# microsoft/UniVL

Measured on AMD Instinct MI355X. Metric: video-text pairs/sec (retrieval finetune, 48x48), higher is better.
Workload: dtype bf16; 1 GPU; YouCookII-shape retrieval finetune (FT-Joint) training step: BERT-base text encoder (12 L) + 6-layer visual encoder, max_words=48, max_frames=48, bs=4 per GPU, fwd+bwd+clip+BertAdam, dropout 0.10, random-init weights; kind=joint, per_gpu_batch=4, global_batch=4, max_words=48, max_frames=48, parallelism=dp1, hip_graph=True, graph_mode=whole, optimizer_pipelined=True, optimizer_riding=True, params=152602880

## Files before the change

### univl_amd/csrc/gemm.hip

```cpp
#include <stdlib.h>
#include "common.h"
#include "univl_hip.h"
#include "adam_body.h"
#include "ln_body.h"

#ifdef UNIVL_TRACE
__device__ unsigned long long* g_univl_trace = nullptr;
__device__ int g_univl_trace_cap = 0;
#define UNIVL_TRACE_AT(phase)                                                                              \
    do {                                                                                                   \
        if (threadIdx.x == 0 && g_univl_trace != nullptr) {                                                \
            const int w__ = blockIdx.x + gridDim.x * (blockIdx.y + gridDim.y * blockIdx.z);                \
            if (w__ < g_univl_trace_cap) g_univl_trace[w__ * 4 + (phase)] = wall_clock64();                \
        }                                                                                                  \
    } while (0)
extern "C" int univl_trace_set(unsigned long long* buf, int cap_workgroups) {
    if (hipMemcpyToSymbol(HIP_SYMBOL(g_univl_trace), &buf, sizeof(buf)) != hipSuccess) return 1;
    if (hipMemcpyToSymbol(HIP_SYMBOL(g_univl_trace_cap), &cap_workgroups, sizeof(int)) != hipSuccess) return 1;
    return 0;
}
#else
#define UNIVL_TRACE_AT(phase)
#endif

// ... 711 lines not shown
    fold_leave(cnt);
}

__host__ __device__ __forceinline__ void pair_tile(int t, int total, int nx, int ny, int nz, int flags, int gm, int& bx, int& by, int& bz) {
    if ((flags & UNIVL_GEMM_XCD_MAP) && total >= 16 && ny > 1) {
        tile_of(xcd_run(t, total), nx, ny, nz, gm, bx, by, bz);
    } else {
        const int nxy = nx * ny;
        bz = t / nxy;
        const int rem = t - bz * nxy;
        by = rem / nx;
        bx = rem - by * nx;
    }
}

template <bool DR, int WF, bool FOLD = false>
__global__ __launch_bounds__(512, (DR && WF == 2 && !FOLD) ? 6 : 4) void gemm_pair_kernel(PairArgs a, LnFold f) {
    const int w0 = blockIdx.x;
    int bx, by, bz;
    if (w0 < a.nd_pad) {
        if (w0 >= a.nd) return;
        pair_tile(w0, a.nd, a.dnx, a.dny, a.dnz, a.d.flags, a.d.gm, bx, by, bz);
        if constexpr (DR) gemm_tile<__bf16, false, true, 64, 128, 2, 2, 4>(a.d, bx, by, bz, a.dnz);
        else gemm_tile<__bf16, false, true, 64, 64, 4, 2, 4>(a.d, bx, by, bz, a.dnz);
        if constexpr (FOLD) ln_fold_bwd(f, by, a.dnx * a.dnz);
    } else if (w0 < a.nd_pad + a.cs.n_pad) {
        const int t = w0 - a.nd_pad;
        if (t >= a.cs.n_tiles) return;
        colsum_tile<512>(a.cs, t, smem_raw);
    } else {
        pair_tile(w0 - a.nd_pad - a.cs.n_pad, a.nw, a.wnx, a.wny, a.wnz, a.w.flags, a.w.gm, bx, by, bz);
        if constexpr (WF == 0) gemm_tile<__bf16, true, true, 64, 64, 4, 2, 4>(a.w, bx, by, bz, a.wnz);
        else if constexpr (WF == 1) gemm_tile<__bf16, true, true, 64, 64, 6, 2, 4>(a.w, bx, by, bz, a.wnz);
        else if constexpr (WF == 2) gemm_tile<__bf16, true, true, 128, 64, 2, 4, 2>(a.w, bx, by, bz, a.wnz);
        else gemm_tile<__bf16, true, true, 128, 64, 6, 4, 2>(a.w, bx, by, bz, a.wnz);
    }
}

template <bool DR, int WF, bool FOLD = false>
int launch_pair(const PairArgs& a, hipStream_t stream, const LnFold* f = nullptr) {
    constexpr size_t smem_d = DR ? 2 * (size_t)(64 + 128) * 64 * sizeof(__bf16) : 2 * (size_t)(64 + 64) * 128 * sizeof(__bf16);
    constexpr size_t smem_w = WF == 0 ? 2 * (size_t)(64 + 64) * 128 * sizeof(__bf16)
                              : WF == 1 ? (size_t)(64 + 64) * 192 * sizeof(__bf16)
                              : WF == 2 ? 2 * (size_t)(128 + 64) * 64 * sizeof(__bf16) : (size_t)(128 + 64) * 192 * sizeof(__bf16);
    constexpr size_t smem = smem_d > smem_w ? smem_d : smem_w;
    static_assert(!FOLD || smem >= 8 * 768 * sizeof(float), "LayerNorm-backward fold needs 24 KB of LDS");
    static bool attr_done[UNIVL_MAX_DEVICES] = {};
    univl_allow_lds(gemm_pair_kernel<DR, WF, FOLD>, smem, attr_done);
    LnFold none = {};
    hipLaunchKernelGGL((gemm_pair_kernel<DR, WF, FOLD>), dim3(a.nd_pad + a.cs.n_pad + a.nw), dim3(512), smem, stream, a, f ? *f : none);
    UNIVL_LAUNCH_CHECK();
    return UNIVL_OK;
}

template <typename T, bool TA, bool TB, int BM, int BN, int NC, int WGM, int WGN>
__device__ __forceinline__ void gemm_acc_only(const T* A, long lda, const T* B, long ldb, int M, int N, int K, int m0, int n0,
                                              f32x4_t (&acc)[BM / WGM / 16][BN / WGN / 16], unsigned char* smem) {
    constexpr int BK = NC * Mma<T>::CH, NT = 64 * WGM * WGN;
    using TileA = Tile<T, TA, BM, BK, NT>;
    using TileB = Tile<T, TB, BN, BK, NT>;
    constexpr int WM = BM / WGM, WN = BN / WGN, MI = WM / 16, NI = WN / 16;
    unsigned char* sA = smem;
    unsigned char* sB = sA + 2 * TileA::BYTES;
    const int tid = threadIdx.x, lane = tid & 63, wave = tid >> 6;
    const int wm0 = (wave / WGN) * WM, wn0 = (wave % WGN) * WN;
#pragma unroll
    for (int a = 0; a < MI; ++a)
#pragma unroll
        for (int b = 0; b < NI; ++b) acc[a][b] = f32x4_t{0.f, 0.f, 0.f, 0.f};
    const T* pa[TileA::PER_THREAD];
    const T* pb[TileB::PER_THREAD];
    TileA::init(pa, A, lda, m0, 0, M, tid);
    TileB::init(pb, B, ldb, n0, 0, N, tid);
    const long stepA = TileA::kstep(lda), stepB = TileB::kstep(ldb);
    const int nfull = K / BK;
    TileA::issue(pa, sA, tid);
    TileB::issue(pb, sB, tid);
    TileA::advance(pa, stepA);
    TileB::advance(pb, stepB);
    __syncthreads();
    for (int t = 0; t < nfull; ++t) {
        const int cur = t & 1;
        if (t + 1 < nfull) {
            TileA::issue(pa, sA + (cur ^ 1) * TileA::BYTES, tid);
            TileB::issue(pb, sB + (cur ^ 1) * TileB::BYTES, tid);
            TileA::advance(pa, stepA);
            TileB::advance(pb, stepB);
        }
        tile_mma<T, TA, TB, MI, NI, NC, TileA, TileB>(sA + cur * TileA::BYTES, sB + cur * TileB::BYTES, wm0, wn0, lane, acc);
        __syncthreads();
    }
}

#include "vocab_ce.h"
#include "vocab_score.h"
#include "attn_body.h"

struct AttnFusedArgs {
    UnivlAttention at;
    int Sk_pad, Sq_pad;
    const __bf16* dY; long lddy;
    const __bf16* W; long ldw;
    int K;
    int n_attn, n_attn_pad;
    GemmArgs w;
    int nw, wnx, wny, wnz;
};

template <int TRIPS, bool DUAL, int NCW>
__global__ __launch_bounds__(256) void attn_bwd_odgrad_kernel(AttnFusedArgs a) {
    const int w0 = blockIdx.x;
    if (w0 < a.n_attn_pad) {
        if (w0 >= a.n_attn) return;
        const int bh = w0 >> 1, role = w0 & 1;
        const int b = bh / a.at.H, h = bh % a.at.H;
        f32x4_t acc[2][2];
        gemm_acc_only<__bf16, false, true, 64, 64, 4, 2, 2>(a.dY + (long)b * a.at.Sq * a.lddy, a.lddy, a.W, a.ldw, a.at.Sq, a.at.H * 64, a.K,
                                                            0, h * 64, acc, smem_raw);
        const int lane = threadIdx.x & 63, wave = threadIdx.x >> 6, g = lane >> 4, i = lane & 15;
        const int wm0 = (wave >> 1) * 32, wn0 = (wave & 1) * 32;
        const int Sq = a.at.Sq, Sq_pad = a.Sq_pad;
        auto dow = [&](void* img_, int pitch) {
            __bf16* img = reinterpret_cast<__bf16*>(img_);
#pragma unroll
            for (int ta = 0; ta < 2; ++ta)
#pragma unroll
                for (int tb = 0; tb < 2; ++tb)
#pragma unroll
                    for (int r = 0; r < 4; ++r) {
                        const int row = wm0 + 16 * ta + 4 * g + r, col = wn0 + 16 * tb + i;
                        if (row < Sq_pad) img[row * pitch + col] = row < Sq ? (__bf16)acc[ta][tb][r] : (__bf16)0.0f;
                    }
        };
        attn_bwd_body<__bf16, TRIPS, DUAL, true>(a.at, a.Sk_pad, a.Sq_pad, 1, 0.125f, bh, role, smem_raw, dow);
    } else {
        int bx, by, bz;
        pair_tile(w0 - a.n_attn_pad, a.nw, a.wnx, a.wny, a.wnz, a.w.flags, a.w.gm, bx, by, bz);
        gemm_tile<__bf16, true, true, 64, 64, NCW, 2, 2>(a.w, bx, by, bz, a.wnz);
    }
}

struct AttnFwdFusedArgs {
    UnivlAttention at;
    int Sk_pad;
    const __bf16* X; long ldx;
    const __bf16* W; long ldw;
    const float* bias;
    __bf16* qkv; long ldqkv;
    int K;
    int n_attn, n_attn_pad;
    const __bf16* X_lo; const __bf16* W_lo;
};

template <bool NT, bool BIG>
__global__ __launch_bounds__(512, 2) void attn_fwd_qkv_kernel(AttnFwdFusedArgs a, UnivlAdam ad, int c0, int c1) {
    const int w0 = blockIdx.x;
    if (w0 >= a.n_attn_pad) {
        const int nb = (int)gridDim.x - a.n_attn_pad;
        for (int c = c0 + (w0 - a.n_attn_pad); c < c1; c += nb) adam_chunk<NT, 512>(ad, c);
        return;
    }
    if (w0 >= a.n_attn) return;
    constexpr int ROWS = BIG ? 128 : 64, MI = ROWS / 32;
    using TileA = Tile<__bf16, false, ROWS, 64, 512>;
    using TileB = Tile<__bf16, false, 192, 64, 512>;
    const int bh = BIG ? (w0 >> 1) : w0, yblk = BIG ? (w0 & 1) : 0, b = bh / a.at.H, h = bh % a.at.H;
    const int HD3 = a.at.H * 64, Sq = a.at.Sq;
    const int tid = threadIdx.x, lane = tid & 63, wave = tid >> 6, g = lane >> 4, i = lane & 15;
    const int wm0 = (wave >> 2) * (ROWS / 2), wn0 = (wave & 3) * 48;
    unsigned char* sA = smem_raw;
    unsigned char* sB = sA + 2 * TileA::BYTES;
    f32x4_t acc[MI][3];
#pragma unroll
    for (int ta = 0; ta < MI; ++ta)
#pragma unroll
        for (int tb = 0; tb < 3; ++tb) acc[ta][tb] = f32x4_t{0.f, 0.f, 0.f, 0.f};
    const __bf16* pa[TileA::PER_THREAD];
    const __bf16* pb[TileB::PER_THREAD];
    TileA::init(pa, a.X + (long)b * Sq * a.ldx, a.ldx, 0, 0, Sq, tid);
#pragma unroll
    for (int c = 0; c < TileB::PER_THREAD; ++c) {
        int r, q;
        TileB::coords(c, tid, r, q);
        pb[c] = a.W + (long)((r >> 6) * HD3 + h * 64 + (r & 63)) * a.ldw + q * 8;
    }
    const int nseg = 1 + (a.W_lo != nullptr ? 1 : 0) + (a.X_lo != nullptr ? 1 : 0);
    const int per = a.K / 64, nfull = nseg * per;
    int seg = 0, wrap = per;
    auto seg_x = [&](int s_) { return (a.X_lo != nullptr && s_ > 0 && s_ == nseg - 1) ? a.X_lo : a.X; };
    auto seg_w = [&](int s_) { return (a.W_lo != nullptr && s_ == 1) ? a.W_lo : a.W; };
    TileA::issue(pa, sA, tid);
    TileB::issue(pb, sB, tid);
    TileA::advance(pa, 64);
    TileB::advance(pb, 64);
    __syncthreads();
    for (int t = 0; t < nfull; ++t) {
        const int cur = t & 1;
        if (t + 1 < nfull) {
            if (t + 1 == wrap) {
                TileA::advance(pa, (seg_x(seg + 1) - seg_x(seg)) - (long)a.K);
                TileB::advance(pb, (seg_w(seg + 1) - seg_w(seg)) - (long)a.K);
                ++seg;
                wrap += per;
            }
            TileA::issue(pa, sA + (cur ^ 1) * TileA::BYTES, tid);
            TileB::issue(pb, sB + (cur ^ 1) * TileB::BYTES, tid);
            TileA::advance(pa, 64);
            TileB::advance(pb, 64);
        }
        tile_mma<__bf16, false, false, MI, 3, 2, TileA, TileB>(sA + cur * TileA::BYTES, sB + cur * TileB::BYTES, wm0, wn0, lane, acc);
        __syncthreads();
    }
    const AttnFwdImages<__bf16> im(smem_raw, a.Sk_pad);
    using C = AttnCfg<__bf16>;
#pragma unroll
    for (int tb = 0; tb < 3; ++tb) {
        const int col = wn0 + 16 * tb + i, panel = col >> 6, c64 = col & 63;
        const int gcol = panel * HD3 + h * 64 + c64;
        const float bv = a.bias ? a.bias[gcol] : 0.0f;
        __bf16* img = panel == 0 ? im.sQ : (panel == 1 ? im.sK : im.sV);
        const int pitch = panel == 2 ? C::PT : C::PK;
#pragma unroll
        for (int ta = 0; ta < MI; ++ta)
#pragma unroll
            for (int r = 0; r < 4; ++r) {
                const int row = wm0 + 16 * ta + 4 * g + r;
                const __bf16 v = (__bf16)(acc[ta][tb][r] * 1.0f + bv);
                if (row < Sq && (!BIG || (row >> 6) == yblk)) a.qkv[((long)b * Sq + row) * a.ldqkv + gcol] = v;
                if (row < a.Sk_pad || (!BIG && panel == 0)) img[row * pitch + c64] = row < Sq ? v : (__bf16)0.0f;
            }
    }
    attn_fwd_body<__bf16, BIG ? 8 : 4, true>(a.at, a.Sk_pad, 0.125f, bh, yblk, smem_raw);
}

template <bool NT>
__global__ __launch_bounds__(512, 2) void gemm_adam_kernel(GemmArgs g, int nd, int nd_pad, int nx, int ny, int nz, UnivlAdam a, int c0, int c1) {
    const int w0 = blockIdx.x;
    if (w0 < nd_pad) {
        if (w0 >= nd) return;
        int bx, by, bz;
        pair_tile(w0, nd, nx, ny, nz, g.flags, g.gm, bx, by, bz);
        gemm_tile<__bf16, false, false, 64, 64, 4, 2, 4, true>(g, bx, by, bz, nz);
    } else {
        const int nb = (int)gridDim.x - nd_pad;
        for (int c = c0 + (w0 - nd_pad); c < c1; c += nb) adam_chunk<NT, 512>(a, c);
    }
}

__host__ __device__ __forceinline__ bool rect_rider_role(int w0, int total, int nd_pad, int& idx) {
    const int gi = w0 >> 3, nrg = (total - nd_pad) >> 3, pg = (total >> 3) / nrg;
    const int k = gi / pg;
    if (gi - k * pg == pg - 1 && k < nrg) { idx = k * 8 + (w0 & 7); return true; }
    idx = w0 - 8 * (k < nrg ? k : nrg);
    return false;
}

template <bool NT>
__global__ __launch_bounds__(512, 6) void gemm_adam_rect_kernel(GemmArgs g, int nd, int nd_pad, int nx, int ny, int nz, UnivlAdam a, int c0, int c1) {
    int t;
    if (rect_rider_role((int)blockIdx.x, (int)gridDim.x, nd_pad, t)) {
        const int nb = (int)gridDim.x - nd_pad;
        for (int c = c0 + t; c < c1; c += nb) adam_chunk<NT, 512, false>(a, c);
    } else {
        if (t >= nd) return;
        int bx, by, bz;
        pair_tile(t, nd, nx, ny, nz, g.flags, g.gm, bx, by, bz);
        gemm_tile<__bf16, false, false, 64, 128, 2, 2, 4>(g, bx, by, bz, nz);
    }
}

__device__ __forceinline__ void ln_fold(const LnFold& f, const int by, const int n, const int M) {
    int* cnt = f.counters + 2 * by;
    const int slab = fold_arrive(cnt, n);
    if (slab < 0) return;
    const int row = by * 64 + slab * 8 + (int)(threadIdx.x >> 6);
    if (row < M) ln_fwd_row<768, __bf16, false, true>(f.ln, row, (int)(threadIdx.x & 63));
    fold_leave(cnt);
}

template <bool NT>
__global__ __launch_bounds__(512, 2) void gemm_ln_kernel(GemmArgs g, int nd, int nd_pad, int nx, int ny, int nz, UnivlAdam a, int c0, int c1, LnFold f) {
    const int w0 = blockIdx.x;
    if (w0 < nd_pad) {
        if (w0 >= nd) return;
        int bx, by, bz;
        pair_tile(w0, nd, nx, ny, nz, g.flags, g.gm, bx, by, bz);
        gemm_tile<__bf16, false, false, 64, 64, 4, 2, 4, true>(g, bx, by, bz, nz);
        ln_fold(f, by, nx * nz, g.M);
    } else {
        const int nb = (int)gridDim.x - nd_pad;
        for (int c = c0 + (w0 - nd_pad); c < c1; c += nb) adam_chunk<NT, 512>(a, c);
    }
}

template <typename T, bool TA, bool TB, int BM, int BN, int NC, int WGM = 2, int WGN = 2>
int launch(const GemmArgs& a, int ksplit, hipStream_t stream) {
    constexpr int BK = NC * Mma<T>::CH, NT = 64 * WGM * WGN;
    using TileA = Tile<T, TA, BM, BK, NT>;
    using TileB = Tile<T, TB, BN, BK, NT>;
    const size_t smem = NC == 6 ? TileA::BYTES + TileB::BYTES : 2 * (TileA::BYTES + TileB::BYTES);
    static bool attr_done[UNIVL_MAX_DEVICES] = {};
    if (smem > 48 * 1024) univl_allow_lds(gemm_kernel<T, TA, TB, BM, BN, NC, WGM, WGN>, smem, attr_done);
    dim3 grid((a.N + BN - 1) / BN, (a.M + BM - 1) / BM, ksplit);
    hipLaunchKernelGGL((gemm_kernel<T, TA, TB, BM, BN, NC, WGM, WGN>), grid, dim3(NT), smem, stream, a);
    UNIVL_LAUNCH_CHECK();
    return UNIVL_OK;
}

template <typename T, int BM, int BN, int NC, int WGM = 2, int WGN = 2>
int dispatch_trans(const GemmArgs& a, int ta, int tb, int ksplit, hipStream_t s) {
    if (!ta && !tb) return launch<T, false, false, BM, BN, NC, WGM, WGN>(a, ksplit, s);
    if (!ta && tb) return launch<T, false, true, BM, BN, NC, WGM, WGN>(a, ksplit, s);
    if (ta && tb) return launch<T, true, true, BM, BN, NC, WGM, WGN>(a, ksplit, s);
    return launch<T, true, false, BM, BN, NC, WGM, WGN>(a, ksplit, s);
}

}

__global__ __launch_bounds__(256) void dot_kernel(GemmArgs p) {
    __shared__ float red[4];
    const int n = blockIdx.x, m = blockIdx.y, t = threadIdx.x;
    const float* a = reinterpret_cast<const float*>(p.A) + (long)m * p.lda;
    const float* b = reinterpret_cast<const float*>(p.B) + (long)n * p.ldb;
    float acc = 0.f;
    const int k4 = p.K & ~3;
    for (int k = 4 * t; k < k4; k += 1024) {
        const float4 x = *reinterpret_cast<const float4*>(a + k);
        const float4 y = *reinterpret_cast<const float4*>(b + k);
        acc += (x.x * y.x + x.y * y.y) + (x.z * y.z + x.w * y.w);
    }
    if (t < p.K - k4) acc += a[k4 + t] * b[k4 + t];
    acc = wave_sum(acc);
    if ((t & 63) == 0) red[t >> 6] = acc;
    __syncthreads();
    if (t == 0) {
        float v = ((red[0] + red[1]) + (red[2] + red[3])) * p.alpha;
        const long o = (long)m * p.ldc + n;
        if (p.flags & UNIVL_GEMM_ACCUM) v += p.C32[o];
        if (p.C32) p.C32[o] = v;
        if (p.C16) reinterpret_cast<float*>(p.C16)[o] = v;
    }
}

struct Choice { int tile, nc, waves; };

constexpr long GEMM_BIG_MIN = 256;
constexpr int GEMM_GM = 8;
constexpr long GEMM_NC64_MIN = 1024;

static bool fits256(const UnivlGemm* d, bool in_group) {
    if (d->dtype != UNIVL_BF16 || (d->trans_a && !d->trans_b) || d->M % 256 != 0 || d->N % 256 != 0) return false;
    if (d->dbias && !in_group) return false;
    if (d->flags & UNIVL_GEMM_AUX_F32) return false;
    if (d->sumsq && d->sumsq_rows % 256 != 0) return false;
    if (d->ldc % 4 != 0 || (d->R && d->ldr % 4 != 0) || (d->aux && d->ldaux % 4 != 0) || !aligned16(d->C32) || !aligned16(d->R) ||
        !aligned16(d->bias) || (((uintptr_t)d->C16 | (uintptr_t)d->aux) & 7) != 0) return false;
    const int ks = (d->ksplit < 1 || univl_deterministic()) ? 1 : d->ksplit;
    return d->K % (128 * ks) == 0;
}

constexpr int G256_MIN_ROWS = 1536;
constexpr long G256_MIN_WG = 192, G256_MAX_WG = 256;
static bool auto256(const UnivlGemm* d, bool in_group) {
    if (!fits256(d, in_group)) return false;
    const int ks = (d->ksplit < 1 || univl_deterministic()) ? 1 : d->ksplit;
    const long wg = (long)(d->M / 256) * (d->N / 256) * ks;
    const int rows = d->trans_a ? d->K : d->M;
    return rows >= G256_MIN_ROWS && (in_group || (ks == 1 && wg >= G256_MIN_WG && wg <= G256_MAX_WG));
}

static Choice choose(const UnivlGemm* d, int forced_tile, int forced_nc = 0, bool allow_rect = false, bool in_group = false) {
    const bool bf16 = d->dtype == UNIVL_BF16;
    int want = forced_tile ? forced_tile : d->tile;
    const bool pairs = d->A_lo || d->B_lo || d->C16_lo;
    if (!pairs && ((want == 256 && fits256(d, in_group)) || (want == 0 && auto256(d, in_group)))) return Choice{256, 2, 8};
    if (want == 256) want = 128;
    const long tiles128 = (long)((d->M + 127) / 128) * ((d->N + 127) / 128);
    const bool rect_ok = allow_rect && bf16 && !d->trans_a && !d->sumsq && !d->dbias;
    Choice c;
    if (want == 12864 || want == 64128) {
        c.tile = rect_ok ? want : 128;
        c.nc = 2;
        c.waves = !rect_ok ? 4 : (d->waves ? d->waves : 8);
        return c;
    }
// ... 155 lines not shown
        if (c.nc == 2) {
            if (c.waves == 8) return dispatch_trans<__bf16, 64, 64, 2, 2, 4>(a, ta, tb, ksplit, stream);
            return dispatch_trans<__bf16, 64, 64, 2>(a, ta, tb, ksplit, stream);
        }
        if (c.waves == 8) return dispatch_trans<__bf16, 64, 64, 4, 2, 4>(a, ta, tb, ksplit, stream);
        return dispatch_trans<__bf16, 64, 64, 4>(a, ta, tb, ksplit, stream);
    }
    if (c.tile == 128) return dispatch_trans<float, 128, 128, 2>(a, ta, tb, ksplit, stream);
    return dispatch_trans<float, 64, 64, 4>(a, ta, tb, ksplit, stream);
}

static bool has_pairs(const UnivlGemm* d) { return d->A_lo != nullptr || d->B_lo != nullptr || d->C16_lo != nullptr; }

static int pair_impl(const UnivlGemm* dgrad, const UnivlGemm* wgrad, const UnivlLayerNorm* ln, int32_t* counters, int32_t dry_run,
                     hipStream_t stream) {
    UNIVL_CHECK_ARG(dgrad != nullptr && wgrad != nullptr, UNIVL_EINVAL, "univl_gemm_pair: null descriptor");
    UNIVL_CHECK_ARG(!has_pairs(dgrad) && !has_pairs(wgrad), UNIVL_EUNSUPPORTED, "univl_gemm_pair: operand pairs are carried by univl_gemm / the rider and fold launches only");
    PairArgs a;
    int ksd, ksw;
    Choice cd, cw;
    int rc = prepare(dgrad, a.d, ksd, cd);
    if (rc != UNIVL_OK) return rc;
    rc = prepare(wgrad, a.w, ksw, cw);
    if (rc != UNIVL_OK) return rc;
    UNIVL_CHECK_ARG(dgrad->dtype == UNIVL_BF16 && wgrad->dtype == UNIVL_BF16 && !dgrad->trans_a && dgrad->trans_b && wgrad->trans_a &&
                        wgrad->trans_b && cd.tile == 64 && cw.tile == 64 && cd.nc == 4 && (cw.nc == 4 || cw.nc == 6) && !dgrad->sumsq,
                    UNIVL_EUNSUPPORTED, "univl_gemm_pair: needs a bf16 (K-major, T-major) product and a bf16 (T-major, T-major) product on the 64 tile");
    const long dslice = ((long)dgrad->K + ksd - 1) / ksd;
    const bool plain = dgrad->tile == 0 && wgrad->tile == 0;
    const bool drect = plain && dgrad->M >= 384 && dslice <= 1536;
    const bool wrect = plain && wgrad->M % 128 == 0 && (!wgrad->sumsq || wgrad->sumsq_rows % 128 == 0);
    const bool wone = cw.nc == 6;
    if (drect) {
        rc = prepare(dgrad, a.d, ksd, cd, 64, 2);
        if (rc != UNIVL_OK) return rc;
        UNIVL_CHECK_ARG(cd.nc == 2, UNIVL_EUNSUPPORTED, "univl_gemm_pair: rectangular dgrad body needs 64-deep K steps");
    }
    if (wrect && !wone) {
        rc = prepare(wgrad, a.w, ksw, cw, 64, 2);
        if (rc != UNIVL_OK) return rc;
        UNIVL_CHECK_ARG(cw.nc == 2, UNIVL_EUNSUPPORTED, "univl_gemm_pair: rectangular weight-gradient body needs 64-deep K steps");
    }
    const int dbn = drect ? 128 : 64, wbm = wrect ? 128 : 64;
    a.dnx = (dgrad->N + dbn - 1) / dbn; a.dny = (dgrad->M + 63) / 64; a.dnz = ksd;
    a.wnx = (wgrad->N + 63) / 64; a.wny = (wgrad->M + wbm - 1) / wbm; a.wnz = ksw;
    a.nd = a.dnx * a.dny * a.dnz;
    a.nd_pad = (a.nd + 7) / 8 * 8;
    a.nw = a.wnx * a.wny * a.wnz;
    a.cs = ColsumArgs{nullptr, 0, 0, 0, nullptr, 0, 0};
    if (wgrad->dbias && wgrad->K <= 2048 && wgrad->M % 8 == 0) {
        a.cs.x = reinterpret_cast<const __bf16*>(wgrad->A);
        a.cs.ld = wgrad->lda;
        a.cs.rows = wgrad->K;
        a.cs.n = wgrad->M;
        a.cs.out = wgrad->dbias;
        a.cs.n_tiles = (wgrad->M + 63) / 64;
        a.cs.n_pad = (a.cs.n_tiles + 7) / 8 * 8;
        a.w.dbias = nullptr;
    }
    if (ln != nullptr) {
        UNIVL_CHECK_ARG(!univl_deterministic() && (!drect || (wrect && !wone)) && counters != nullptr && dgrad->C32 && !dgrad->C16 && dgrad->N == 768 &&
                            dgrad->ldc == 768 && !(dgrad->flags & (UNIVL_GEMM_GELU_FWD | UNIVL_GEMM_GELU_BWD | UNIVL_GEMM_ACCUM)) &&
                            a.dnx * a.dnz >= LN_SHARE && a.dny <= LN_FOLD_MAX_BLOCKS && ln->dtype == UNIVL_BF16 && ln->N == 768 && ln->rows == dgrad->M &&
                            ln->dout == (const float*)dgrad->C32 && ln->gamma && ln->y && ln->stats && !ln->dpos &&
                            (const void*)ln->dx32 != (const void*)dgrad->C32,
                        UNIVL_EUNSUPPORTED, "univl_gemm_pair_ln: not a (dgrad, LayerNorm backward) pair this launch carries");
        a.d.flags |= UNIVL_GEMM_ATOMIC;
    }
    if (dry_run) return UNIVL_OK;
    if (ln != nullptr) {
        LnFold f;
        f.ln = *ln;
        f.counters = counters;
        if (drect) return launch_pair<true, 2, true>(a, stream, &f);
        if (wrect) return wone ? launch_pair<false, 3, true>(a, stream, &f) : launch_pair<false, 2, true>(a, stream, &f);
        return wone ? launch_pair<false, 1, true>(a, stream, &f) : launch_pair<false, 0, true>(a, stream, &f);
    }
    if (drect) return wrect ? launch_pair<true, 2>(a, stream) : launch_pair<true, 0>(a, stream);
    if (wrect) return wone ? launch_pair<false, 3>(a, stream) : launch_pair<false, 2>(a, stream);
    return wone ? launch_pair<false, 1>(a, stream) : launch_pair<false, 0>(a, stream);
}

extern "C" int univl_gemm_pair(const UnivlGemm* dgrad, const UnivlGemm* wgrad, int32_t dry_run, hipStream_t stream) {
    UNIVL_ON_STREAM_DEVICE(stream);
    return pair_impl(dgrad, wgrad, nullptr, nullptr, dry_run, stream);
}

extern "C" int univl_gemm_pair_ln(const UnivlGemm* dgrad, const UnivlGemm* wgrad, const UnivlLayerNorm* ln, int32_t* counters,
                                  int32_t dry_run, hipStream_t stream) {
    UNIVL_ON_STREAM_DEVICE(stream);
    UNIVL_CHECK_ARG(ln != nullptr && counters != nullptr, UNIVL_EINVAL, "univl_gemm_pair_ln: null argument");
    return pair_impl(dgrad, wgrad, ln, counters, dry_run, stream);
}

extern "C" int univl_attention_bwd_fused(const UnivlAttention* at, const UnivlGemm* odgrad, const UnivlGemm* owgrad, int32_t dry_run,
                                         hipStream_t stream) {
    UNIVL_ON_STREAM_DEVICE(stream);
    UNIVL_CHECK_ARG(at != nullptr && odgrad != nullptr, UNIVL_EINVAL, "univl_attention_bwd_fused: null descriptor");
    int rc = attn_check(at, "univl_attention_bwd_fused", true);
    if (rc) return rc;
    using C = AttnCfg<__bf16>;
    const int Sk_pad = (at->Sk + 31) / 32 * 32, Sq_pad = (at->Sq + 31) / 32 * 32;
    const UnivlGemm* g = odgrad;
    UNIVL_CHECK_ARG(at->dtype == UNIVL_DT_BF16 && Sk_pad <= 64 && Sq_pad <= 64 && g->dtype == UNIVL_BF16 && !g->trans_a && g->trans_b &&
                        g->M == at->B * at->Sq && g->N == at->H * 64 && g->K % 128 == 0 && g->K >= 128 && g->C16 == at->dout && !g->C32 &&
                        g->ldc == at->lddo && !g->bias && !g->R && !g->dbias && !g->sumsq && g->alpha == 1.0f && g->ksplit <= 1 &&
                        (g->flags & ~(UNIVL_GEMM_XCD_MAP)) == 0 && aligned16(g->A) && aligned16(g->B) && g->lda % 8 == 0 && g->ldb % 8 == 0 &&
                        !g->A_lo && !g->B_lo && !g->C16_lo,
                    UNIVL_EUNSUPPORTED, "univl_attention_bwd_fused: not an (attention backward, attention-output dgrad) pair this launch carries");
    AttnFusedArgs a;
    a.at = *at;
    a.Sk_pad = Sk_pad; a.Sq_pad = Sq_pad;
    a.dY = reinterpret_cast<const __bf16*>(g->A); a.lddy = g->lda;
    a.W = reinterpret_cast<const __bf16*>(g->B); a.ldw = g->ldb;
    a.K = g->K;
    a.n_attn = 2 * at->B * at->H;
    a.n_attn_pad = (a.n_attn + 7) / 8 * 8;
    a.nw = 0; a.wnx = a.wny = a.wnz = 1;
    bool wone = false;
    if (owgrad != nullptr) {
        int ksw;
        Choice cw;
        rc = prepare(owgrad, a.w, ksw, cw);
        if (rc != UNIVL_OK) return rc;
        UNIVL_CHECK_ARG(owgrad->dtype == UNIVL_BF16 && owgrad->trans_a && owgrad->trans_b && cw.tile == 64 && (cw.nc == 4 || cw.nc == 6) &&
                            !owgrad->dbias, UNIVL_EUNSUPPORTED, "univl_attention_bwd_fused: the riding weight gradient must be a bf16 (T-major, T-major) product on the 64 tile");
        wone = cw.nc == 6;
        a.wnx = (owgrad->N + 63) / 64; a.wny = (owgrad->M + 63) / 64; a.wnz = ksw;
        a.nw = a.wnx * a.wny * a.wnz;
    } else {
        a.w = GemmArgs{};
    }
    if (dry_run) return UNIVL_OK;
    constexpr bool DUAL = true;
    const size_t smemA = (size_t)Sk_pad * (C::PT + 2 * C::PK) * 2 + Sk_pad * 4 + 64 * C::PK * 2;
    const size_t smemB = (size_t)Sq_pad * (2 * C::PT + 2 * C::PK) * 2 + (Sk_pad + 2 * Sq_pad) * 4;
    size_t smem = 4 * (size_t)64 * 128 * 2;
    smem = smem > smemA ? smem : smemA;
    smem = smem > smemB ? smem : smemB;
    constexpr int TR = (64 * 8 + 511) / 512;
    static bool done4[UNIVL_MAX_DEVICES] = {}, done6[UNIVL_MAX_DEVICES] = {};
    const dim3 grid(a.n_attn_pad + a.nw);
    if (wone) {
        univl_allow_lds(attn_bwd_odgrad_kernel<TR, DUAL, 6>, 160 * 1024, done6);
        hipLaunchKernelGGL((attn_bwd_odgrad_kernel<TR, DUAL, 6>), grid, dim3(256), smem, stream, a);
    } else {
        univl_allow_lds(attn_bwd_odgrad_kernel<TR, DUAL, 4>, 160 * 1024, done4);
        hipLaunchKernelGGL((attn_bwd_odgrad_kernel<TR, DUAL, 4>), grid, dim3(256), smem, stream, a);
    }
    UNIVL_LAUNCH_CHECK();
    return UNIVL_OK;
}

static const size_t ATTN_FWD_FUSED_SMEM = 2 * (size_t)(64 + 192) * 64 * sizeof(__bf16);
static const size_t ATTN_FWD_FUSED_SMEM_BIG = 2 * (size_t)(128 + 192) * 64 * sizeof(__bf16);
static void attn_fwd_fused_allow_lds() {
    static bool done_nt[UNIVL_MAX_DEVICES] = {}, done_t[UNIVL_MAX_DEVICES] = {}, done_ntb[UNIVL_MAX_DEVICES] = {}, done_tb[UNIVL_MAX_DEVICES] = {};
    univl_allow_lds(attn_fwd_qkv_kernel<true, false>, ATTN_FWD_FUSED_SMEM, done_nt);
    univl_allow_lds(attn_fwd_qkv_kernel<false, false>, ATTN_FWD_FUSED_SMEM, done_t);
    univl_allow_lds(attn_fwd_qkv_kernel<true, true>, ATTN_FWD_FUSED_SMEM_BIG, done_ntb);
    univl_allow_lds(attn_fwd_qkv_kernel<false, true>, ATTN_FWD_FUSED_SMEM_BIG, done_tb);
}

extern "C" int univl_attention_fwd_fused(const UnivlAttention* at, const UnivlGemm* qkv, const UnivlAdam* adam, int32_t chunk_begin,
                                         int32_t chunk_count, int32_t max_blocks, int32_t dry_run, hipStream_t stream) {
    UNIVL_ON_STREAM_DEVICE(stream);
    UNIVL_CHECK_ARG(at != nullptr && qkv != nullptr, UNIVL_EINVAL, "univl_attention_fwd_fused: null descriptor");
    int rc = adam_range_check("univl_attention_fwd_fused", adam, chunk_begin, chunk_count, true);
    if (rc) return rc;
    rc = attn_check(at, "univl_attention_fwd_fused", false);
    if (rc) return rc;
    const int Sk_pad = (at->Sk + 31) / 32 * 32;
    const UnivlGemm* g = qkv;
    const long hd = (long)at->H * 64;
    const __bf16* c16 = reinterpret_cast<const __bf16*>(g->C16);
    UNIVL_CHECK_ARG(at->dtype == UNIVL_DT_BF16 && at->Sq == at->Sk && Sk_pad <= 128 && !at->causal && at->bsk == 0 && at->bsv == 0 &&
                        g->dtype == UNIVL_BF16 && !g->trans_a && !g->trans_b && g->M == at->B * at->Sq && g->N == 3 * hd && g->K % 64 == 0 &&
                        g->K >= 64 && c16 != nullptr && !g->C32 && !g->R && !g->dbias && !g->sumsq && !g->aux && g->alpha == 1.0f &&
                        g->ksplit <= 1 && (g->flags & ~(UNIVL_GEMM_XCD_MAP)) == 0 && aligned16(g->A) && aligned16(g->B) && g->lda % 8 == 0 &&
                        aligned16(g->A_lo) && aligned16(g->B_lo) && !g->C16_lo &&
                        g->ldb % 8 == 0 && at->q == (const void*)c16 && at->k == (const void*)(c16 + hd) && at->v == (const void*)(c16 + 2 * hd) &&
                        at->ldq == g->ldc && at->ldk == g->ldc && at->ldv == g->ldc,
                    UNIVL_EUNSUPPORTED, "univl_attention_fwd_fused: not a (q|k|v projection, self-attention) pair this launch carries");
    if (dry_run) return UNIVL_OK;
    AttnFwdFusedArgs a;
    a.at = *at;
    a.Sk_pad = Sk_pad;
    a.X = reinterpret_cast<const __bf16*>(g->A); a.ldx = g->lda;
    a.W = reinterpret_cast<const __bf16*>(g->B); a.ldw = g->ldb;
    a.bias = g->bias;
    a.qkv = reinterpret_cast<__bf16*>(g->C16); a.ldqkv = g->ldc;
    a.K = g->K;
    a.X_lo = reinterpret_cast<const __bf16*>(g->A_lo); a.W_lo = reinterpret_cast<const __bf16*>(g->B_lo);
    const bool big = Sk_pad > 64;
    a.n_attn = at->B * at->H * (big ? 2 : 1);
    a.n_attn_pad = (a.n_attn + 7) / 8 * 8;
    const AdamRange r = adam_range(adam, chunk_begin, chunk_count, max_blocks);
    attn_fwd_fused_allow_lds();
    const dim3 grid(a.n_attn_pad + r.blocks);
    adam_with_nt([&](auto nt) {
        constexpr bool NT = decltype(nt)::value;
        if (big) hipLaunchKernelGGL((attn_fwd_qkv_kernel<NT, true>), grid, dim3(512), ATTN_FWD_FUSED_SMEM_BIG, stream, a, r.adam, r.c0, r.c1);
        else hipLaunchKernelGGL((attn_fwd_qkv_kernel<NT, false>), grid, dim3(512), ATTN_FWD_FUSED_SMEM, stream, a, r.adam, r.c0, r.c1);
    });
    UNIVL_LAUNCH_CHECK();
    return UNIVL_OK;
}

static const size_t RIDER_SMEM = 4 * (size_t)Tile<__bf16, false, 64, 128, 512>::BYTES;
static void rider_allow_lds() {
    static bool done_nt[UNIVL_MAX_DEVICES] = {}, done_t[UNIVL_MAX_DEVICES] = {};
    univl_allow_lds(gemm_adam_kernel<true>, RIDER_SMEM, done_nt);
    univl_allow_lds(gemm_adam_kernel<false>, RIDER_SMEM, done_t);
}

static int rider_form(const UnivlGemm* gemm, const Choice& c) {
    if (gemm->dtype != UNIVL_BF16 || gemm->trans_a || gemm->trans_b || gemm->sumsq || gemm->dbias) return 0;
    if (c.tile == 64 && c.nc == 4) return 1;
    if (c.tile == 64128 && c.waves == 8) return 2;
    return 0;
}

static int rider_prepare(const UnivlGemm* gemm, GemmArgs& a, int& ks, int& form) {
    Choice c;
    int rc = prepare(gemm, a, ks, c);
    if (rc != UNIVL_OK) return rc;
    form = rider_form(gemm, c);
    if (form == 0) {
        rc = prepare(gemm, a, ks, c, 0, 0, true);
        if (rc != UNIVL_OK) return rc;
        form = rider_form(gemm, c);
    }
    return UNIVL_OK;
}

extern "C" int univl_gemm_rider_fits(const UnivlGemm* gemm) {
    UNIVL_CHECK_ARG(gemm != nullptr, UNIVL_EINVAL, "univl_gemm_rider_fits: null descriptor");
    GemmArgs a;
    int ks, form;
    const int rc = rider_prepare(gemm, a, ks, form);
    if (rc != UNIVL_OK) return rc;
    return form != 0 ? 1 : 0;
}

extern "C" int univl_gemm_rider(const UnivlGemm* gemm, const UnivlAdam* adam, int32_t chunk_begin, int32_t chunk_count,
                                int32_t max_blocks, hipStream_t stream) {
    UNIVL_ON_STREAM_DEVICE(stream);
    UNIVL_CHECK_ARG(gemm != nullptr, UNIVL_EINVAL, "univl_gemm_rider: null descriptor");
    int rc = adam_range_check("univl_gemm_rider", adam, chunk_begin, chunk_count, false);
    if (rc != UNIVL_OK) return rc;
    GemmArgs a;
    int ks, fits;
    rc = rider_prepare(gemm, a, ks, fits);
    if (rc != UNIVL_OK) return rc;
    if (fits == 2 && adam->p16_lo != nullptr) fits = 0;
    if (!fits || chunk_count == 0) {
        const int r1 = univl_gemm(gemm, stream);
        if (r1 != UNIVL_OK || chunk_count == 0) return r1;
        return univl_bert_adam_range(adam, chunk_begin, chunk_count, 0, max_blocks, stream);
    }
    const int nx = (gemm->N + (fits == 2 ? 127 : 63)) / (fits == 2 ? 128 : 64), ny = (gemm->M + 63) / 64;
    const int nd = nx * ny * ks, nd_pad = (nd + 7) / 8 * 8;
    const AdamRange r = adam_range(adam, chunk_begin, chunk_count, max_blocks);
    if (fits == 2) {
        constexpr size_t smem = 2 * (size_t)(64 + 128) * 64 * sizeof(__bf16);
        const int nb8 = (r.blocks + 7) / 8 * 8;
        adam_with_nt([&](auto nt) {
            hipLaunchKernelGGL(gemm_adam_rect_kernel<decltype(nt)::value>, dim3(nd_pad + nb8), dim3(512), smem, stream, a, nd, nd_pad, nx, ny,
                               ks, r.adam, r.c0, r.c1);
        });
        UNIVL_LAUNCH_CHECK();
        return UNIVL_OK;
    }
    rider_allow_lds();
    adam_with_nt([&](auto nt) {
        hipLaunchKernelGGL(gemm_adam_kernel<decltype(nt)::value>, dim3(nd_pad + r.blocks), dim3(512), RIDER_SMEM, stream, a, nd, nd_pad, nx, ny,
                           ks, r.adam, r.c0, r.c1);
    });
    UNIVL_LAUNCH_CHECK();
    return UNIVL_OK;
}

static void gemm_ln_allow_lds() {
    static bool done_nt[UNIVL_MAX_DEVICES] = {}, done_t[UNIVL_MAX_DEVICES] = {};
    univl_allow_lds(gemm_ln_kernel<true>, RIDER_SMEM, done_nt);
    univl_allow_lds(gemm_ln_kernel<false>, RIDER_SMEM, done_t);
}

extern "C" int univl_gemm_ln(const UnivlGemm* gemm, const UnivlLayerNorm* ln, int32_t* counters, const UnivlAdam* adam,
                             int32_t chunk_begin, int32_t chunk_count, int32_t max_blocks, int32_t dry_run, hipStream_t stream) {
    UNIVL_ON_STREAM_DEVICE(stream);
    UNIVL_CHECK_ARG(gemm != nullptr && ln != nullptr && counters != nullptr, UNIVL_EINVAL, "univl_gemm_ln: null argument");
    int rc = adam_range_check("univl_gemm_ln", adam, chunk_begin, chunk_count, true);
    if (rc != UNIVL_OK) return rc;
    GemmArgs a;
    int ks;
    Choice c;
    rc = prepare(gemm, a, ks, c);
    if (rc != UNIVL_OK) return rc;
    const int nx = (gemm->N + 63) / 64, ny = (gemm->M + 63) / 64;
    UNIVL_CHECK_ARG(!univl_deterministic() && gemm->dtype == UNIVL_BF16 && !gemm->trans_a && !gemm->trans_b && c.tile == 64 && c.nc == 4 &&
                        !gemm->sumsq && !gemm->dbias && gemm->C32 && !gemm->C16 && gemm->N == 768 && gemm->ldc == 768 &&
                        !(gemm->flags & (UNIVL_GEMM_GELU_FWD | UNIVL_GEMM_GELU_BWD | UNIVL_GEMM_ACCUM)) && nx * ks >= LN_SHARE &&
                        ny <= LN_FOLD_MAX_BLOCKS && ln->dtype == UNIVL_BF16 && ln->N == 768 && ln->rows == gemm->M && !ln->x_f64 &&
                        ln->x == (const void*)gemm->C32 && ln->gamma && ln->beta && (ln->out16 || ln->out32),
                    UNIVL_EUNSUPPORTED, "univl_gemm_ln: not a (product, LayerNorm) pair this launch carries");
    if (dry_run) return UNIVL_OK;
    a.flags |= UNIVL_GEMM_ATOMIC;
    const int nd = nx * ny * ks, nd_pad = (nd + 7) / 8 * 8;
    const AdamRange r = adam_range(adam, chunk_begin, chunk_count, max_blocks);
    LnFold f;
    f.ln = *ln;
    f.counters = counters;
    gemm_ln_allow_lds();
    adam_with_nt([&](auto nt) {
        hipLaunchKernelGGL(gemm_ln_kernel<decltype(nt)::value>, dim3(nd_pad + r.blocks), dim3(512), RIDER_SMEM, stream, a, nd, nd_pad, nx, ny,
                           ks, r.adam, r.c0, r.c1, f);
    });
    UNIVL_LAUNCH_CHECK();
    return UNIVL_OK;
}

extern "C" int univl_gemm_rider_prime(hipStream_t stream) {
    UNIVL_ON_STREAM_DEVICE(stream);
    rider_allow_lds();
    attn_fwd_fused_allow_lds();
    gemm_ln_allow_lds();
    return UNIVL_OK;
}

#ifdef UNIVL_PROTO
struct ProtoArgs {
    int n_o, n_o_pad, onx, ony, onz;
    int n_f1, n_f1_pad, f1nx, f1ny;
    int n_f2, f2nx, f2ny, f2nz;
    int* flags1; int* flags2;
};

__device__ __forceinline__ void proto_raise(int* flag) {
    asm volatile("s_waitcnt vmcnt(0)" ::: "memory");
    __syncthreads();
    if (threadIdx.x == 0) __hip_atomic_fetch_add(flag, 1, __ATOMIC_RELAXED, __HIP_MEMORY_SCOPE_AGENT);
}
__device__ __forceinline__ void proto_wait(int* flag, int need) {
    if (threadIdx.x == 0) {
        int polls = 0;
        while (__hip_atomic_load(flag, __ATOMIC_RELAXED, __HIP_MEMORY_SCOPE_AGENT) < need && ++polls < (1 << 22)) __builtin_amdgcn_s_sleep(1);
    }
    __syncthreads();
}

__global__ __launch_bounds__(512, 2) void layer_ffn_proto_kernel(GemmArgs o, GemmArgs f1, GemmArgs f2, LnFold ln1, LnFold ln2, ProtoArgs q) {
    const int w0 = blockIdx.x;
    int bx, by, bz;
    if (w0 < q.n_o_pad) {
        if (w0 >= q.n_o) return;
// ... 267 lines not shown
```

Measured before the change: 1853 pairs/s.

## Deepen fused QKV-projection attention prologue to a four-stage async load ring

Adds a configurable multi-stage (default four) LDS ring for the QKV projection GEMM inside the fused attention-forward kernel, replacing the double buffer with counted vmcnt waits so more global loads stay in flight. The small (64-row) form uses the ring only when the attention workgroups plus Adam rider blocks fit the CU count. The larger LDS footprint drops occupancy to one workgroup per CU for that variant. Trace hooks are also added.

```diff
diff --git a/univl_amd/csrc/gemm.hip b/univl_amd/csrc/gemm.hip
--- a/univl_amd/csrc/gemm.hip
+++ b/univl_amd/csrc/gemm.hip
@@ -887,24 +887,48 @@
     const __bf16* X_lo; const __bf16* W_lo;
 };
 
-template <bool NT, bool BIG>
-__global__ __launch_bounds__(512, 2) void attn_fwd_qkv_kernel(AttnFwdFusedArgs a, UnivlAdam ad, int c0, int c1) {
+#ifndef UNIVL_ATTN_QKV_STAGES
+#define UNIVL_ATTN_QKV_STAGES 4
+#endif
+struct AttnFwdQkv {
+    static constexpr int RING = UNIVL_ATTN_QKV_STAGES;
+    static constexpr int STAGE_BYTES = (64 + 192) * 64 * (int)sizeof(__bf16);
+    static constexpr int STAGE_BYTES_BIG = (128 + 192) * 64 * (int)sizeof(__bf16);
+    static constexpr int LOADS = STAGE_BYTES / 16 / 512;
+    static constexpr size_t smem(bool big, int ns) { return (size_t)ns * (big ? STAGE_BYTES_BIG : STAGE_BYTES); }
+    static constexpr int wgs_per_cu(bool big, int ns) { return smem(big, ns) <= 80 * 1024 ? 2 : 1; }
+    static_assert(RING >= 2 && RING <= 4, "ring depth");
+};
+__device__ __forceinline__ void attn_qkv_wait_dma(const int n) {
+    static_assert(AttnFwdQkv::LOADS == 4 && AttnFwdQkv::RING <= 4, "the counted waits below: four DMA instructions per stage, at most two stages behind");
+    if (n >= 8) asm volatile("s_waitcnt vmcnt(8)" ::: "memory");
+    else if (n == 4) asm volatile("s_waitcnt vmcnt(4)" ::: "memory");
+    else asm volatile("s_waitcnt vmcnt(0)" ::: "memory");
+}
+
+template <bool NT, bool BIG, int NS>
+__global__ __launch_bounds__(512, AttnFwdQkv::wgs_per_cu(BIG, NS)) void attn_fwd_qkv_kernel(AttnFwdFusedArgs a, UnivlAdam ad, int c0, int c1) {
     const int w0 = blockIdx.x;
     if (w0 >= a.n_attn_pad) {
         const int nb = (int)gridDim.x - a.n_attn_pad;
+        UNIVL_TRACE_AT(0);
         for (int c = c0 + (w0 - a.n_attn_pad); c < c1; c += nb) adam_chunk<NT, 512>(ad, c);
+        UNIVL_TRACE_AT(3);
         return;
     }
     if (w0 >= a.n_attn) return;
     constexpr int ROWS = BIG ? 128 : 64, MI = ROWS / 32;
+    static_assert(NS == 2 || !BIG, "the 128-row form has two stages");
     using TileA = Tile<__bf16, false, ROWS, 64, 512>;
     using TileB = Tile<__bf16, false, 192, 64, 512>;
+    static_assert(TileA::PER_THREAD + TileB::PER_THREAD == AttnFwdQkv::LOADS || BIG, "DMA instructions per stage");
     const int bh = BIG ? (w0 >> 1) : w0, yblk = BIG ? (w0 & 1) : 0, b = bh / a.at.H, h = bh % a.at.H;
     const int HD3 = a.at.H * 64, Sq = a.at.Sq;
     const int tid = threadIdx.x, lane = tid & 63, wave = tid >> 6, g = lane >> 4, i = lane & 15;
     const int wm0 = (wave >> 2) * (ROWS / 2), wn0 = (wave & 3) * 48;
+    UNIVL_TRACE_AT(0);
     unsigned char* sA = smem_raw;
-    unsigned char* sB = sA + 2 * TileA::BYTES;
+    unsigned char* sB = sA + NS * TileA::BYTES;
     f32x4_t acc[MI][3];
 #pragma unroll
     for (int ta = 0; ta < MI; ++ta)
@@ -924,28 +948,50 @@
     int seg = 0, wrap = per;
     auto seg_x = [&](int s_) { return (a.X_lo != nullptr && s_ > 0 && s_ == nseg - 1) ? a.X_lo : a.X; };
     auto seg_w = [&](int s_) { return (a.W_lo != nullptr && s_ == 1) ? a.W_lo : a.W; };
-    TileA::issue(pa, sA, tid);
-    TileB::issue(pb, sB, tid);
-    TileA::advance(pa, 64);
-    TileB::advance(pb, 64);
-    __syncthreads();
-    for (int t = 0; t < nfull; ++t) {
-        const int cur = t & 1;
-        if (t + 1 < nfull) {
-            if (t + 1 == wrap) {
-                TileA::advance(pa, (seg_x(seg + 1) - seg_x(seg)) - (long)a.K);
-                TileB::advance(pb, (seg_w(seg + 1) - seg_w(seg)) - (long)a.K);
-                ++seg;
-                wrap += per;
+    auto issue_stage = [&](const int s, const int slot) {
+        if (s == wrap) {
+            TileA::advance(pa, (seg_x(seg + 1) - seg_x(seg)) - (long)a.K);
+            TileB::advance(pb, (seg_w(seg + 1) - seg_w(seg)) - (long)a.K);
+            ++seg;
+            wrap += per;
+        }
+        TileA::issue(pa, sA + slot * TileA::BYTES, tid);
+        TileB::issue(pb, sB + slot * TileB::BYTES, tid);
+        TileA::advance(pa, 64);
+        TileB::advance(pb, 64);
+    };
+    if constexpr (NS == 2) {
+        issue_stage(0, 0);
+        __syncthreads();
+        UNIVL_TRACE_AT(1);
+        for (int t = 0; t < nfull; ++t) {
+            const int cur = t & 1;
+            if (t + 1 < nfull) issue_stage(t + 1, cur ^ 1);
+            tile_mma<__bf16, false, false, MI, 3, 2, TileA, TileB>(sA + cur * TileA::BYTES, sB + cur * TileB::BYTES, wm0, wn0, lane, acc);
+            __syncthreads();
+        }
+    } else {
+        int issued = 0;
+        for (; issued < NS - 1 && issued < nfull; ++issued) issue_stage(issued, issued);
+        int cur = 0, nxt = NS - 1;
+        for (int t = 0; t < nfull; ++t) {
+            attn_qkv_wait_dma((issued - 1 - t) * AttnFwdQkv::LOADS);
+            asm volatile("s_waitcnt lgkmcnt(0)" ::: "memory");
+            __builtin_amdgcn_s_barrier();
+            asm volatile("" ::: "memory");
+            if (t == 0) UNIVL_TRACE_AT(1);
+            if (issued < nfull) {
+                issue_stage(issued, nxt);
+                ++issued;
             }
-            TileA::issue(pa, sA + (cur ^ 1) * TileA::BYTES, tid);
-            TileB::issue(pb, sB + (cur ^ 1) * TileB::BYTES, tid);
-            TileA::advance(pa, 64);
-            TileB::advance(pb, 64);
-        }
-        tile_mma<__bf16, false, false, MI, 3, 2, TileA, TileB>(sA + cur * TileA::BYTES, sB + cur * TileB::BYTES, wm0, wn0, lane, acc);
+            tile_mma<__bf16, false, false, MI, 3, 2, TileA, TileB>(sA + cur * TileA::BYTES, sB + cur * TileB::BYTES, wm0, wn0, lane, acc);
+            asm volatile("" ::: "memory");
+            cur = cur + 1 == NS ? 0 : cur + 1;
+            nxt = nxt + 1 == NS ? 0 : nxt + 1;
+        }
         __syncthreads();
     }
+    UNIVL_TRACE_AT(2);
     const AttnFwdImages<__bf16> im(smem_raw, a.Sk_pad);
     using C = AttnCfg<__bf16>;
 #pragma unroll
@@ -966,6 +1012,7 @@
             }
     }
     attn_fwd_body<__bf16, BIG ? 8 : 4, true>(a.at, a.Sk_pad, 0.125f, bh, yblk, smem_raw);
+    UNIVL_TRACE_AT(3);
 }
 
 template <bool NT>
@@ -1427,14 +1474,29 @@
     return UNIVL_OK;
 }
 
-static const size_t ATTN_FWD_FUSED_SMEM = 2 * (size_t)(64 + 192) * 64 * sizeof(__bf16);
-static const size_t ATTN_FWD_FUSED_SMEM_BIG = 2 * (size_t)(128 + 192) * 64 * sizeof(__bf16);
+template <bool NT, bool BIG, int NS> static void attn_fwd_qkv_allow_lds() {
+    static bool done[UNIVL_MAX_DEVICES] = {};
+    univl_allow_lds(attn_fwd_qkv_kernel<NT, BIG, NS>, AttnFwdQkv::smem(BIG, NS), done);
+}
+template <bool NT, bool BIG, int NS>
+static void attn_fwd_qkv_launch(const dim3 grid, hipStream_t stream, const AttnFwdFusedArgs& a, const AdamRange& r) {
+    attn_fwd_qkv_allow_lds<NT, BIG, NS>();
+    hipLaunchKernelGGL((attn_fwd_qkv_kernel<NT, BIG, NS>), grid, dim3(512), AttnFwdQkv::smem(BIG, NS), stream, a, r.adam, r.c0, r.c1);
+}
 static void attn_fwd_fused_allow_lds() {
-    static bool done_nt[UNIVL_MAX_DEVICES] = {}, done_t[UNIVL_MAX_DEVICES] = {}, done_ntb[UNIVL_MAX_DEVICES] = {}, done_tb[UNIVL_MAX_DEVICES] = {};
-    univl_allow_lds(attn_fwd_qkv_kernel<true, false>, ATTN_FWD_FUSED_SMEM, done_nt);
-    univl_allow_lds(attn_fwd_qkv_kernel<false, false>, ATTN_FWD_FUSED_SMEM, done_t);
-    univl_allow_lds(attn_fwd_qkv_kernel<true, true>, ATTN_FWD_FUSED_SMEM_BIG, done_ntb);
-    univl_allow_lds(attn_fwd_qkv_kernel<false, true>, ATTN_FWD_FUSED_SMEM_BIG, done_tb);
+    attn_fwd_qkv_allow_lds<true, false, 2>();
+    attn_fwd_qkv_allow_lds<false, false, 2>();
+    attn_fwd_qkv_allow_lds<true, false, AttnFwdQkv::RING>();
+    attn_fwd_qkv_allow_lds<false, false, AttnFwdQkv::RING>();
+    attn_fwd_qkv_allow_lds<true, true, 2>();
+    attn_fwd_qkv_allow_lds<false, true, 2>();
+}
+static int attn_fwd_fused_units() {
+    static int units[UNIVL_MAX_DEVICES] = {};
+    int dev = 0, n = 0;
+    if (hipGetDevice(&dev) != hipSuccess || dev < 0 || dev >= UNIVL_MAX_DEVICES) return 0;
+    if (units[dev] == 0 && hipDeviceGetAttribute(&n, hipDeviceAttributeMultiprocessorCount, dev) == hipSuccess) units[dev] = n;
+    return units[dev];
 }
 
 extern "C" int univl_attention_fwd_fused(const UnivlAttention* at, const UnivlGemm* qkv, const UnivlAdam* adam, int32_t chunk_begin,
@@ -1471,12 +1533,14 @@
     a.n_attn = at->B * at->H * (big ? 2 : 1);
     a.n_attn_pad = (a.n_attn + 7) / 8 * 8;
     const AdamRange r = adam_range(adam, chunk_begin, chunk_count, max_blocks);
-    attn_fwd_fused_allow_lds();
     const dim3 grid(a.n_attn_pad + r.blocks);
+    const int free_units = attn_fwd_fused_units() - a.n_attn_pad;
+    const bool ring = !big && AttnFwdQkv::RING > 2 && free_units >= 0 && r.blocks <= 2 * free_units;
     adam_with_nt([&](auto nt) {
         constexpr bool NT = decltype(nt)::value;
-        if (big) hipLaunchKernelGGL((attn_fwd_qkv_kernel<NT, true>), grid, dim3(512), ATTN_FWD_FUSED_SMEM_BIG, stream, a, r.adam, r.c0, r.c1);
-        else hipLaunchKernelGGL((attn_fwd_qkv_kernel<NT, false>), grid, dim3(512), ATTN_FWD_FUSED_SMEM, stream, a, r.adam, r.c0, r.c1);
+        if (big) attn_fwd_qkv_launch<NT, true, 2>(grid, stream, a, r);
+        else if (ring) attn_fwd_qkv_launch<NT, false, AttnFwdQkv::RING>(grid, stream, a, r);
+        else attn_fwd_qkv_launch<NT, false, 2>(grid, stream, a, r);
     });
     UNIVL_LAUNCH_CHECK();
     return UNIVL_OK;
```

Result: faster. 1889 pairs/s, median of 6 (+2.0%).
